# gongweibao/FleetX

Hardware: AMD Instinct MI355X
Metric: tokens/sec (whole node) GPT-3 6.7B hybrid-parallel at 1/2/4/8 MI355X (higher is better)
Workload: dtype bf16; 1 GPU; model=gpt3-6.7B, global_batch=8, seq_len=1024, parallelism=dp1, micro_batch=8, hip_graph=True, grad_reduce_dtype=float32, recompute=False

## Files before the change

csrc/kernels/norm_eltwise.hip:

```cpp
#include "fx_common.h"

namespace {

struct DropCfg {
  uint32_t klo, khi, thr;
  float scale;
  int enabled;
  const uint64_t* salt;
};

__device__ __forceinline__ DropCfg resolve_drop(DropCfg d) {
  if (d.enabled && d.salt != nullptr) {
    const uint64_t k = salt_key(((uint64_t)d.khi << 32) | d.klo, *d.salt);
    d.klo = (uint32_t)k;
    d.khi = (uint32_t)(k >> 32);
  }
  return d;
}

__device__ __forceinline__ float drop_apply(float v, uint64_t idx, const DropCfg& d) {
  if (!d.enabled) return v;
  uint32_t h = elem_rand_pair(idx, d.klo, d.khi);
  uint32_t r = (idx & 1) ? (h >> 16) : (h & 0xffffu);
  return r >= d.thr ? v * d.scale : 0.f;
// ... 129 lines not shown
      drop_apply8(v, base + c, drop);
    if (residual) {
      float r[8];
      load8<T>(residual + base + c, r);
      for (int j = 0; j < 8; ++j) v[j] += r[j];
    }
  };
  float sum = 0.f;
  for (int vi = lane; vi < nv; vi += 64) {
    float v[8];
    value(vi * 8, v);
    if (s_out) {
      store8<T>(s_out + base + vi * 8, v);
      for (int j = 0; j < 8; ++j) v[j] = round_to<T>(v[j]);
    }
    for (int j = 0; j < 8; ++j) sum += v[j];
  }
  const float mean = wave_sum(sum) / h;
  float var = 0.f;
  for (int vi = lane; vi < nv; vi += 64) {
    float v[8];
    if (s_out) load8<T>(s_out + base + vi * 8, v); else value(vi * 8, v);
    for (int j = 0; j < 8; ++j) { float d = v[j] - mean; var += d * d; }
  }
  const float rstd = rsqrtf(wave_sum(var) / h + eps);
  for (int vi = lane; vi < nv; vi += 64) {
    float v[8], g[8], b[8], o[8];
    if (s_out) load8<T>(s_out + base + vi * 8, v); else value(vi * 8, v);
    load8<T>(gamma + vi * 8, g);
    load8<T>(beta + vi * 8, b);
    for (int j = 0; j < 8; ++j) o[j] = (v[j] - mean) * rstd * g[j] + b[j];
    store8<T>(y + base + vi * 8, o);
  }
  if (lane == 0) { mean_out[row] = mean; rstd_out[row] = rstd; }
}

template <typename T, int VPT, bool MASK = false>
__global__ __launch_bounds__(256) void ln_bwd_row_kernel(
    const uint16_t* __restrict__ dy, const uint16_t* __restrict__ s,
    const float* __restrict__ mean_in, const float* __restrict__ rstd_in,
    const uint16_t* __restrict__ gamma, const uint16_t* __restrict__ ds_in,
    uint16_t* __restrict__ ds_out, uint16_t* __restrict__ dx_out, int rows, int h,
    DropCfg drop_) {
  const DropCfg drop = resolve_drop(drop_);
  const int lane = threadIdx.x & 63;
  const int row = blockIdx.x * 4 + (threadIdx.x >> 6);
  if (row >= rows) return;
  const size_t base = (size_t)row * h;
  const float mean = mean_in[row], rstd = rstd_in[row];
  float xh[VPT][8], gdy[VPT][8];
  float s1 = 0.f, s2 = 0.f;
#pragma unroll
  for (int i = 0; i < VPT; ++i) {
    const int c = (i * 64 + lane) * 8;
    if (MASK && c >= h) {
#pragma unroll
      for (int j = 0; j < 8; ++j) xh[i][j] = gdy[i][j] = 0.f;
      continue;
    }
    float a[8], g[8], d[8];
    load8<T>(s + base + c, a);
    load8<T>(gamma + c, g);
    load8<T>(dy + base + c, d);
#pragma unroll
    for (int j = 0; j < 8; ++j) {
      xh[i][j] = (a[j] - mean) * rstd;
      gdy[i][j] = d[j] * g[j];
      s1 += gdy[i][j];
      s2 += gdy[i][j] * xh[i][j];
    }
  }
  uint4 dr[VPT];
  if (ds_in) {
#pragma unroll
    for (int i = 0; i < VPT; ++i) {
      const int c = (i * 64 + lane) * 8;
      dr[i] = make_uint4(0, 0, 0, 0);
      if (!MASK || c < h) dr[i] = *reinterpret_cast<const uint4*>(ds_in + base + c);
    }
  }
  const float m1 = wave_sum(s1) / h, m2 = wave_sum(s2) / h;
#pragma unroll
  for (int i = 0; i < VPT; ++i) {
    const int c = (i * 64 + lane) * 8;
    if (MASK && c >= h) continue;
    float o[8];
#pragma unroll
    for (int j = 0; j < 8; ++j) o[j] = rstd * (gdy[i][j] - m1 - xh[i][j] * m2);
    if (ds_in) {
      float r[8];
      unpack8<T>(dr[i], r);
#pragma unroll
      for (int j = 0; j < 8; ++j) o[j] += r[j];
    }
    store8<T>(ds_out + base + c, o);
    if (drop.enabled) {
      drop_apply8(o, base + c, drop);
      store8<T>(dx_out + base + c, o);
    } else if (dx_out != ds_out) {
      store8<T>(dx_out + base + c, o);
    }
  }
}

template <typename T>
__global__ __launch_bounds__(256) void ln_bwd_row_generic(
    const uint16_t* __restrict__ dy, const uint16_t* __restrict__ s,
    const float* __restrict__ mean_in, const float* __restrict__ rstd_in,
    const uint16_t* __restrict__ gamma, const uint16_t* __restrict__ ds_in,
    uint16_t* __restrict__ ds_out, uint16_t* __restrict__ dx_out, int rows, int h,
    DropCfg drop_) {
  const DropCfg drop = resolve_drop(drop_);
  const int lane = threadIdx.x & 63;
  const int row = blockIdx.x * 4 + (threadIdx.x >> 6);
  if (row >= rows) return;
  const size_t base = (size_t)row * h;
  const float mean = mean_in[row], rstd = rstd_in[row];
  const int nv = h / 8;
  float s1 = 0.f, s2 = 0.f;
  for (int vi = lane; vi < nv; vi += 64) {
    float a[8], g[8], d[8];
    load8<T>(s + base + vi * 8, a);
    load8<T>(gamma + vi * 8, g);
    load8<T>(dy + base + vi * 8, d);
    for (int j = 0; j < 8; ++j) {
      float xh = (a[j] - mean) * rstd, gd = d[j] * g[j];
      s1 += gd;
      s2 += gd * xh;
    }
  }
  const float m1 = wave_sum(s1) / h, m2 = wave_sum(s2) / h;
  for (int vi = lane; vi < nv; vi += 64) {
    const int c = vi * 8;
    float a[8], g[8], d[8], o[8];
    load8<T>(s + base + c, a);
    load8<T>(gamma + c, g);
    load8<T>(dy + base + c, d);
    for (int j = 0; j < 8; ++j) o[j] = rstd * (d[j] * g[j] - m1 - (a[j] - mean) * rstd * m2);
    if (ds_in) {
      float r[8];
      load8<T>(ds_in + base + c, r);
      for (int j = 0; j < 8; ++j) o[j] += r[j];
    }
    store8<T>(ds_out + base + c, o);
    if (drop.enabled) {
      drop_apply8(o, base + c, drop);
      store8<T>(dx_out + base + c, o);
    } else if (dx_out != ds_out) {
      store8<T>(dx_out + base + c, o);
    }
  }
}

template <typename T, int VPT, int WPR, bool MASK, bool DB>
__global__ __launch_bounds__(256, 2) void ln_bwd_cols_kernel(
    const uint16_t* __restrict__ dy, const uint16_t* __restrict__ s,
    const float* __restrict__ mean_in, const float* __restrict__ rstd_in,
    const uint16_t* __restrict__ gamma, const uint16_t* __restrict__ ds_in,
    uint16_t* __restrict__ ds_out, uint16_t* __restrict__ dx_out, int rows, int h,
    int rows_per_group, float* __restrict__ part, DropCfg drop_) {
  constexpr int NG = 4 / WPR;
  __shared__ float red[4 * 512 * VPT];
  __shared__ float xs[2][4][2];
  const DropCfg drop = resolve_drop(drop_);
  const int lane = threadIdx.x & 63, w = threadIdx.x >> 6;
  const int grp = w / WPR, half = w % WPR;
  const int hw = h / WPR, cbase = half * hw;
  const int r0 = min(rows, (blockIdx.x * NG + grp) * rows_per_group);
  const int r1 = min(rows, r0 + rows_per_group);
  uint4 gp[VPT];
  float ag[VPT][8], ab[VPT][8], ax[DB ? VPT : 1][8];
#pragma unroll
  for (int i = 0; i < VPT; ++i) {
    const int c = (i * 64 + lane) * 8;
    gp[i] = (!MASK || c < hw) ? *reinterpret_cast<const uint4*>(gamma + cbase + c)
                              : make_uint4(0, 0, 0, 0);
#pragma unroll
    for (int j = 0; j < 8; ++j) {
      ag[i][j] = ab[i][j] = 0.f;
      if (DB) ax[i][j] = 0.f;
    }
  }
  for (int k = 0; k < rows_per_group; ++k) {
    const int r = r0 + k;
    const bool live = r < r1;
    if (WPR == 1 && !live) break;
    const size_t base = (size_t)(live ? r : 0) * h + cbase;
    uint4 ca[VPT], cd[VPT], cr[VPT];
    float mean = 0.f, rstd = 0.f, s1 = 0.f, s2 = 0.f;
    if (live) {
#pragma unroll
      for (int i = 0; i < VPT; ++i) {
        const int c = (i * 64 + lane) * 8;
        if (MASK && c >= hw) continue;
        ca[i] = *reinterpret_cast<const uint4*>(s + base + c);
        cd[i] = *reinterpret_cast<const uint4*>(dy + base + c);
      }
      if (ds_in) {
#pragma unroll
        for (int i = 0; i < VPT; ++i) {
          const int c = (i * 64 + lane) * 8;
          if (MASK && c >= hw) continue;
          cr[i] = *reinterpret_cast<const uint4*>(ds_in + base + c);
        }
      }
      mean = mean_in[r];
      rstd = rstd_in[r];
#pragma unroll
      for (int i = 0; i < VPT; ++i) {
        const int c = (i * 64 + lane) * 8;
        if (MASK && c >= hw) continue;
        float a[8], d[8], g[8];
        unpack8<T>(ca[i], a);
        unpack8<T>(cd[i], d);
        unpack8<T>(gp[i], g);
#pragma unroll
        for (int j = 0; j < 8; ++j) {
          const float xh = (a[j] - mean) * rstd, gd = d[j] * g[j];
          s1 += gd;
          s2 += gd * xh;
          ag[i][j] += d[j] * xh;
          ab[i][j] += d[j];
        }
      }
    }
    s1 = wave_sum(s1);
    s2 = wave_sum(s2);
    if constexpr (WPR > 1) {
      if (lane == 0) {
        xs[k & 1][w][0] = s1;
        xs[k & 1][w][1] = s2;
      }
      __syncthreads();
      s1 = xs[k & 1][WPR * grp][0];
      s2 = xs[k & 1][WPR * grp][1];
#pragma unroll
      for (int q = 1; q < WPR; ++q) {
        s1 += xs[k & 1][WPR * grp + q][0];
        s2 += xs[k & 1][WPR * grp + q][1];
      }
    }
    if (!live) continue;
    const float m1 = s1 / h, m2 = s2 / h;
#pragma unroll
    for (int i = 0; i < VPT; ++i) {
      const int c = (i * 64 + lane) * 8;
      if (MASK && c >= hw) continue;
      float a[8], d[8], g[8], o[8];
      unpack8<T>(ca[i], a);
      unpack8<T>(cd[i], d);
      unpack8<T>(gp[i], g);
#pragma unroll
      for (int j = 0; j < 8; ++j) o[j] = rstd * (d[j] * g[j] - m1 - (a[j] - mean) * rstd * m2);
      if (ds_in) {
        float rr[8];
        unpack8<T>(cr[i], rr);
#pragma unroll
        for (int j = 0; j < 8; ++j) o[j] += rr[j];
      }
      store8<T>(ds_out + base + c, o);
      if (drop.enabled) {
        drop_apply8(o, base + c, drop);
        store8<T>(dx_out + base + c, o);
      } else if (dx_out != ds_out) {
        store8<T>(dx_out + base + c, o);
      }
      if (DB) {
#pragma unroll
        for (int j = 0; j < 8; ++j) ax[i][j] += round_to<T>(o[j]);
      }
    }
  }
#pragma unroll
  for (int arr = 0; arr < (DB ? 3 : 2); ++arr) {
    __syncthreads();
#pragma unroll
    for (int i = 0; i < VPT; ++i) {
      const int c = (i * 64 + lane) * 8;
      if (MASK && c >= hw) continue;
#pragma unroll
      for (int j = 0; j < 8; ++j)
        red[grp * h + cbase + c + j] = arr == 0 ? ag[i][j] : arr == 1 ? ab[i][j] : ax[DB ? i : 0][j];
    }
    __syncthreads();
    float* out = part + ((size_t)arr * gridDim.x + blockIdx.x) * h;
    for (int c = threadIdx.x; c < h; c += 256) {
      float v = red[c];
#pragma unroll
      for (int q = 1; q < NG; ++q) v += red[q * h + c];
      out[c] = v;
    }
  }
}

struct LnColsOut {
  float* f32[3];
  uint16_t* t16[3];
  int acc[3];
};
template <typename T>
__global__ __launch_bounds__(256) void ln_cols_finalize_kernel(const float* __restrict__ part,
                                                               int G, int h, LnColsOut f) {
  __shared__ float tr[8][132];
  const int arr = blockIdx.y;
  const float* p = part + (size_t)arr * G * h;
  const int q = threadIdx.x & 31, sr = threadIdx.x >> 5;
  const int c0 = blockIdx.x * 128 + q * 4;
  floatx4 acc = {0.f, 0.f, 0.f, 0.f};
  if (c0 < h) {
    for (int k0 = sr; k0 < G; k0 += 128) {
      floatx4 v[16];
#pragma unroll
      for (int u = 0; u < 16; ++u) {
        const int k = k0 + 8 * u;
        v[u] = k < G ? *reinterpret_cast<const floatx4*>(p + (size_t)k * h + c0)
                     : floatx4{0.f, 0.f, 0.f, 0.f};
      }
#pragma unroll
      for (int u = 0; u < 16; ++u) acc += v[u];
    }
  }
#pragma unroll
  for (int j = 0; j < 4; ++j) tr[sr][q * 4 + j] = acc[j];
  __syncthreads();
  const int c = threadIdx.x, gc = blockIdx.x * 128 + c;
  if (c >= 128 || gc >= h) return;
  float sum = 0.f;
#pragma unroll
  for (int t = 0; t < 8; ++t) sum += tr[t][c];
  if (f.f32[arr]) f.f32[arr][gc] = f.acc[arr] ? f.f32[arr][gc] + sum : sum;
  if (f.t16[arr]) f.t16[arr][gc] = Elt<T>::from_f(sum);
}

typedef __attribute__((address_space(1))) float gf32;
typedef __attribute__((address_space(1))) int gi32;

__device__ __forceinline__ void st_part(float* p, float v) {
  __hip_atomic_store((gf32*)p, v, __ATOMIC_RELAXED, __HIP_MEMORY_SCOPE_AGENT);
}

struct ColFin {
  int* cnt;
  float* f32[2];
  uint16_t* t16[2];
  int acc[2];
};

template <typename T>
__device__ __forceinline__ void colsum_tail(const float* __restrict__ p0,
                                            const float* __restrict__ p1, int cols, int np,
                                            const ColFin& f) {
  __shared__ int last;
  asm volatile("s_waitcnt vmcnt(0)" ::: "memory");
  __syncthreads();
  if (threadIdx.x == 0) {
    const int t = __hip_atomic_fetch_add((gi32*)(f.cnt + 32 * blockIdx.x), 1, __ATOMIC_RELAXED,
                                         __HIP_MEMORY_SCOPE_AGENT);
    last = t == (int)gridDim.y - 1;
    if (last)
      __hip_atomic_store((gi32*)(f.cnt + 32 * blockIdx.x), 0, __ATOMIC_RELAXED,
                         __HIP_MEMORY_SCOPE_AGENT);
  }
  __syncthreads();
  if (!last) return;
  __builtin_amdgcn_fence(__ATOMIC_ACQUIRE, "wavefront");
  __shared__ float tr[8][132];
  const int q = threadIdx.x & 31, sr = threadIdx.x >> 5;
  const int c0 = blockIdx.x * 128 + q * 4;
  const int splits = gridDim.y;
  for (int which = 0; which < np; ++which) {
    const float* p = which ? p1 : p0;
    floatx4 s = {0.f, 0.f, 0.f, 0.f};
    if (c0 < cols) {
      const auto rs = __builtin_amdgcn_make_buffer_rsrc(const_cast<float*>(p), 0,
                                                        splits * cols * 4, 0x00020000);
      for (int k0 = sr; k0 < splits; k0 += 128) {
        floatx4 v[16];
#pragma unroll
        for (int u = 0; u < 16; ++u) {
          const int k = k0 + 8 * u;
          const uint32_t off = k < splits ? (uint32_t)(k * cols + c0) * 4u : 0x80000000u;
          v[u] = __builtin_bit_cast(floatx4, __builtin_amdgcn_raw_buffer_load_b128(rs, off, 0, 16));
        }
#pragma unroll
        for (int u = 0; u < 16; ++u) s += v[u];
      }
    }
#pragma unroll
    for (int j = 0; j < 4; ++j) tr[sr][q * 4 + j] = s[j];
    __syncthreads();
    const int c = threadIdx.x, gc = blockIdx.x * 128 + c;
    if (c < 128 && gc < cols) {
      float sum = 0.f;
#pragma unroll
      for (int t = 0; t < 8; ++t) sum += tr[t][c];
      if (f.f32[which]) f.f32[which][gc] = f.acc[which] ? f.f32[which][gc] + sum : sum;
      if (f.t16[which]) f.t16[which][gc] = Elt<T>::from_f(sum);
    }
    __syncthreads();
  }
}

template <typename T, int MODE>
__global__ __launch_bounds__(256) void coltile_partial_kernel(
    const uint16_t* __restrict__ a, const uint16_t* __restrict__ b,
    const float* __restrict__ mean, const float* __restrict__ rstd,
    float* __restrict__ p0, float* __restrict__ p1, int rows, int cols, int rows_per_split,
    ColFin fin) {
  __shared__ float red[2][16][129];
  const int tx = threadIdx.x & 15, ty = threadIdx.x >> 4;
  const int col = blockIdx.x * 128 + tx * 8;
  const int r0 = blockIdx.y * rows_per_split;
  const int r1 = min(rows, r0 + rows_per_split);
  float acc0[8], acc1[8];
#pragma unroll
  for (int j = 0; j < 8; ++j) acc0[j] = acc1[j] = 0.f;
  if (col < cols) {
    int r = r0 + ty;
    for (; r + 48 < r1; r += 64) {
      float va[4][8], vb[MODE == 0 ? 4 : 1][8], m[4], rs[4];
#pragma unroll
      for (int q = 0; q < 4; ++q) {
        const size_t off = (size_t)(r + 16 * q) * cols + col;
        load8<T>(a + off, va[q]);
        if (MODE == 0) {
          load8<T>(b + off, vb[q]);
          m[q] = mean[r + 16 * q];
          rs[q] = rstd[r + 16 * q];
        }
      }
#pragma unroll
      for (int q = 0; q < 4; ++q) {
#pragma unroll
        for (int j = 0; j < 8; ++j) {
          if (MODE == 0) {
            acc0[j] += va[q][j] * (vb[MODE == 0 ? q : 0][j] - m[q]) * rs[q];
            acc1[j] += va[q][j];
          } else {
            acc0[j] += va[q][j];
          }
        }
      }
    }
    for (; r < r1; r += 16) {
      const size_t off = (size_t)r * cols + col;
// ... 217 lines not shown
    drop_apply8(a, (uint64_t)off, drop);
    store8<T>(y + off, a);
  }
}

DropCfg make_drop(float p, uint64_t key) {
  DropCfg d;
  d.enabled = p > 0.f ? 1 : 0;
  d.klo = (uint32_t)(key & 0xffffffffu);
  d.khi = (uint32_t)(key >> 32);
  d.thr = (uint32_t)(p * 65536.0f + 0.5f);
  d.scale = p < 1.f ? 1.f / (1.f - p) : 0.f;
  d.salt = g_fx_dropout_salt;
  return d;
}

inline int grid_for(long n8) {
  long g = (n8 + 255) / 256;
  if (g > 8192) g = 8192;
  if (g < 1) g = 1;
  return (int)g;
}

inline int splits_for(int rows, int cols) {
  static const int blocks = [] {
    const char* e = getenv("FLEETX_COLSUM_BLOCKS");
    const int v = e ? atoi(e) : 0;
    return v > 0 ? v : 1024;
  }();
  int tiles = (cols + 127) / 128;
  int s = blocks / (tiles > 0 ? tiles : 1);
  if (s < 1) s = 1;
  int max_s = (rows + 15) / 16;
  if (s > max_s) s = max_s;
  if (s > 512) s = 512;
  return s;
}

}

#define FX_DISPATCH_T(dtype, ...)        \
  if (dtype == 0) {                      \
    using T = bf16;                      \
    __VA_ARGS__;                         \
  } else {                               \
    using T = f16;                       \
    __VA_ARGS__;                         \
  }

static ColFin make_fin(int* cnt, float* f0, void* t0, int acc0, float* f1, void* t1, int acc1) {
  ColFin f;
  f.cnt = cnt;
  f.f32[0] = f0; f.f32[1] = f1;
  f.t16[0] = (uint16_t*)t0; f.t16[1] = (uint16_t*)t1;
  f.acc[0] = acc0; f.acc[1] = acc1;
  return f;
}

extern "C" int fx_coltile_splits(int rows, int cols) { return splits_for(rows, cols); }

extern "C" void fx_add_ln_fwd(int dtype, const void* x, const void* bias, const void* residual,
                              const void* gamma, const void* beta, void* s_out, void* y,
                              float* mean, float* rstd, int rows, int h, float eps, float p,
                              uint64_t key, hipStream_t st) {
  DropCfg d = make_drop(p, key);
  dim3 grid((rows + 3) / 4), block(256);
  auto X = (const uint16_t*)x;
  auto B = (const uint16_t*)bias;
  auto R = (const uint16_t*)residual;
  auto G = (const uint16_t*)gamma;
  auto Be = (const uint16_t*)beta;
  auto S = (uint16_t*)s_out;
  auto Y = (uint16_t*)y;
#define LN_CASE(V)                                                                          \
  case V:                                                                                   \
    FX_DISPATCH_T(dtype, add_ln_fwd_kernel<T, V><<<grid, block, 0, st>>>(                   \
                             X, B, R, G, Be, S, Y, mean, rstd, rows, h, eps, d));           \
    break;
  if (h % 512 == 0 && h / 512 <= 16) {
    switch (h / 512) {
      LN_CASE(1) LN_CASE(2) LN_CASE(3) LN_CASE(4) LN_CASE(5) LN_CASE(6) LN_CASE(7) LN_CASE(8)
      LN_CASE(10) LN_CASE(12) LN_CASE(16)
      default:
        FX_DISPATCH_T(dtype, add_ln_fwd_generic<T><<<grid, block, 0, st>>>(
                                 X, B, R, G, Be, S, Y, mean, rstd, rows, h, eps, d));
    }
  } else if (h % 8 == 0 && h < 8 * 512) {
#define LNM_CASE(V)                                                                          \
  case V:                                                                                    \
    FX_DISPATCH_T(dtype, add_ln_fwd_kernel<T, V, true><<<grid, block, 0, st>>>(              \
                             X, B, R, G, Be, S, Y, mean, rstd, rows, h, eps, d));            \
    break;
    switch ((h + 511) / 512) {
      LNM_CASE(1) LNM_CASE(2) LNM_CASE(3) LNM_CASE(4) LNM_CASE(5) LNM_CASE(6) LNM_CASE(7)
      LNM_CASE(8)
    }
#undef LNM_CASE
  } else {
    FX_DISPATCH_T(dtype, add_ln_fwd_generic<T><<<grid, block, 0, st>>>(
                             X, B, R, G, Be, S, Y, mean, rstd, rows, h, eps, d));
  }
#undef LN_CASE
}

extern "C" void fx_ln_bwd_row(int dtype, const void* dy, const void* s, const float* mean,
                              const float* rstd, const void* gamma, const void* ds_in,
                              void* ds_out, void* dx_out, int rows, int h, float p, uint64_t key,
                              hipStream_t st) {
  DropCfg d = make_drop(p, key);
  dim3 grid((rows + 3) / 4), block(256);
  auto DY = (const uint16_t*)dy;
  auto S = (const uint16_t*)s;
  auto G = (const uint16_t*)gamma;
  auto DI = (const uint16_t*)ds_in;
  auto DS = (uint16_t*)ds_out;
  auto DX = (uint16_t*)dx_out;
#define LNB_CASE(V)                                                                       \
  case V:                                                                                 \
    FX_DISPATCH_T(dtype, ln_bwd_row_kernel<T, V><<<grid, block, 0, st>>>(                 \
                             DY, S, mean, rstd, G, DI, DS, DX, rows, h, d));              \
    break;
  if (h % 512 == 0 && h / 512 <= 8) {
    switch (h / 512) {
      LNB_CASE(1) LNB_CASE(2) LNB_CASE(3) LNB_CASE(4) LNB_CASE(5) LNB_CASE(6) LNB_CASE(7)
      LNB_CASE(8)
      default:
        FX_DISPATCH_T(dtype, ln_bwd_row_generic<T><<<grid, block, 0, st>>>(
                                 DY, S, mean, rstd, G, DI, DS, DX, rows, h, d));
    }
  } else if (h % 8 == 0 && h < 8 * 512) {
#define LNBM_CASE(V)                                                                      \
  case V:                                                                                 \
    FX_DISPATCH_T(dtype, ln_bwd_row_kernel<T, V, true><<<grid, block, 0, st>>>(           \
                             DY, S, mean, rstd, G, DI, DS, DX, rows, h, d));              \
    break;
    switch ((h + 511) / 512) {
      LNBM_CASE(1) LNBM_CASE(2) LNBM_CASE(3) LNBM_CASE(4) LNBM_CASE(5) LNBM_CASE(6)
      LNBM_CASE(7) LNBM_CASE(8)
    }
#undef LNBM_CASE
  } else {
    FX_DISPATCH_T(dtype, ln_bwd_row_generic<T><<<grid, block, 0, st>>>(
                             DY, S, mean, rstd, G, DI, DS, DX, rows, h, d));
  }
#undef LNB_CASE
}

static int ln_cols_wpr(int h) { return h <= 1536 ? 1 : h <= 3072 ? 2 : 4; }
static int ln_cols_rows_per_group(int rows, int h) {
  const int ng = 4 / ln_cols_wpr(h);
  int rpg = (rows + 512 * ng - 1) / (512 * ng);
  return rpg < 2 ? 2 : rpg;
}
extern "C" int fx_ln_bwd_cols_blocks(int rows, int h, int max_h) {
  if (rows <= 0 || h > (max_h < 4096 ? max_h : 4096) || h % (8 * ln_cols_wpr(h))) return 0;
  const int ng = 4 / ln_cols_wpr(h), rpg = ln_cols_rows_per_group(rows, h);
  return (rows + ng * rpg - 1) / (ng * rpg);
}

extern "C" int fx_ln_bwd_cols(int dtype, const void* dy, const void* s, const float* mean,
                              const float* rstd, const void* gamma, const void* ds_in,
                              void* ds_out, void* dx_out, int rows, int h, float p, uint64_t key,
                              float* part, int with_dbias, float* fg, void* tg, int accg,
                              float* fb, void* tb, int accb, float* fx, void* tx, int accx,
                              hipStream_t st) {
  const int G = fx_ln_bwd_cols_blocks(rows, h, 4096);
  if (G == 0) return -1;
  const int wpr = ln_cols_wpr(h), hw = h / wpr;
  const int rpg = ln_cols_rows_per_group(rows, h);
  DropCfg d = make_drop(p, key);
  auto DY = (const uint16_t*)dy;
  auto S = (const uint16_t*)s;
  auto GM = (const uint16_t*)gamma;
  auto DI = (const uint16_t*)ds_in;
  auto DS = (uint16_t*)ds_out;
  auto DX = (uint16_t*)dx_out;
  const int vpt = (hw + 511) / 512;
  const bool mask = hw % 512 != 0;
#define LNC_GO(V, W, M, DB)                                                                   \
  FX_DISPATCH_T(dtype, ln_bwd_cols_kernel<T, V, W, M, DB><<<G, 256, 0, st>>>(                 \
                           DY, S, mean, rstd, GM, DI, DS, DX, rows, h, rpg, part, d))
#define LNC_M(V, W)                                                                           \
  if (mask) {                                                                                 \
    if (with_dbias) { LNC_GO(V, W, true, true); } else { LNC_GO(V, W, true, false); }         \
  } else {                                                                                    \
    if (with_dbias) { LNC_GO(V, W, false, true); } else { LNC_GO(V, W, false, false); }       \
  }
#define LNC_V(V)                                                                              \
  case V:                                                                                     \
    if (wpr == 1) { LNC_M(V, 1) } else if (wpr == 2) { LNC_M(V, 2) } else { LNC_M(V, 4) }     \
    break;
  switch (vpt) {
    LNC_V(1) LNC_V(2) LNC_V(3)
    default: return -1;
  }
#undef LNC_V
#undef LNC_M
#undef LNC_GO
  LnColsOut f;
  f.f32[0] = fg; f.f32[1] = fb; f.f32[2] = fx;
  f.t16[0] = (uint16_t*)tg; f.t16[1] = (uint16_t*)tb; f.t16[2] = (uint16_t*)tx;
  f.acc[0] = accg; f.acc[1] = accb; f.acc[2] = accx;
  dim3 grid((h + 127) / 128, with_dbias ? 3 : 2);
  FX_DISPATCH_T(dtype, ln_cols_finalize_kernel<T><<<grid, 256, 0, st>>>(part, G, h, f));
  return 0;
}

extern "C" void fx_coltile_partial(int dtype, int mode, const void* a, const void* b,
                                   const float* mean, const float* rstd, float* p0, float* p1,
                                   int rows, int cols, int splits, hipStream_t st, int* cnt,
                                   float* f0, void* t0, int acc0, float* f1, void* t1, int acc1) {
  const ColFin fin = make_fin(cnt, f0, t0, acc0, f1, t1, acc1);
  int rps = (rows + splits - 1) / splits;
  dim3 grid((cols + 127) / 128, splits), block(256);
  auto A = (const uint16_t*)a;
  auto B = (const uint16_t*)b;
  if (mode == 0) {
    FX_DISPATCH_T(dtype, coltile_partial_kernel<T, 0><<<grid, block, 0, st>>>(
                             A, B, mean, rstd, p0, p1, rows, cols, rps, fin));
  } else {
    FX_DISPATCH_T(dtype, coltile_partial_kernel<T, 1><<<grid, block, 0, st>>>(
                             A, B, mean, rstd, p0, p1, rows, cols, rps, fin));
  }
}

extern "C" void fx_coltile_finalize(int dtype, const float* part, int splits, int cols,
                                    float* out_f32, void* out_t, int accumulate, hipStream_t st) {
  dim3 grid((cols + 255) / 256), block(256);
  FX_DISPATCH_T(dtype, coltile_finalize_kernel<T><<<grid, block, 0, st>>>(
                           part, splits, cols, out_f32, (uint16_t*)out_t, accumulate));
}

extern "C" void fx_bias_gelu_fwd(int dtype, int erf, const void* x, const void* bias, void* y,
                                 long n, int cols, hipStream_t st) {
  long n8 = n / 8;
  if (erf) {
    FX_DISPATCH_T(dtype, bias_gelu_fwd_kernel<T, true><<<grid_for(n8), 256, 0, st>>>(
                             (const uint16_t*)x, (const uint16_t*)bias, (uint16_t*)y, n8, cols));
  } else {
    FX_DISPATCH_T(dtype, bias_gelu_fwd_kernel<T, false><<<grid_for(n8), 256, 0, st>>>(
                             (const uint16_t*)x, (const uint16_t*)bias, (uint16_t*)y, n8, cols));
  }
}

extern "C" void fx_bias_gelu_bwd(int dtype, int erf, const void* dy, const void* x,
                                 const void* bias, void* dx, float* part, int rows, int cols,
                                 int splits, hipStream_t st, int* cnt, float* out_f32,
                                 void* out_t, int acc) {
  const ColFin fin = make_fin(cnt, out_f32, out_t, acc, nullptr, nullptr, 0);
  int rps = (rows + splits - 1) / splits;
  dim3 grid((cols + 127) / 128, splits), block(256);
  if (erf) {
    FX_DISPATCH_T(dtype, bias_gelu_bwd_kernel<T, true><<<grid, block, 0, st>>>(
                             (const uint16_t*)dy, (const uint16_t*)x, (const uint16_t*)bias,
                             (uint16_t*)dx, part, rows, cols, rps, fin));
  } else {
    FX_DISPATCH_T(dtype, bias_gelu_bwd_kernel<T, false><<<grid, block, 0, st>>>(
                             (const uint16_t*)dy, (const uint16_t*)x, (const uint16_t*)bias,
                             (uint16_t*)dx, part, rows, cols, rps, fin));
  }
}

extern "C" void fx_bias_dropout_add_fwd(int dtype, const void* x, const void* bias,
                                        const void* residual, void* out, long n, int cols, float p,
                                        uint64_t key, hipStream_t st) {
  DropCfg d = make_drop(p, key);
  long n8 = n / 8;
  FX_DISPATCH_T(dtype, bias_dropout_add_fwd_kernel<T><<<grid_for(n8), 256, 0, st>>>(
                           (const uint16_t*)x, (const uint16_t*)bias, (const uint16_t*)residual,
                           (uint16_t*)out, n8, cols, d));
}

extern "C" void fx_dropout_bwd_colsum(int dtype, const void* dout, void* dx, float* part,
                                      int rows, int cols, int splits, float p, uint64_t key,
                                      hipStream_t st, int* cnt, float* out_f32, void* out_t,
                                      int acc) {
  const ColFin fin = make_fin(cnt, out_f32, out_t, acc, nullptr, nullptr, 0);
  DropCfg d = make_drop(p, key);
  int rps = (rows + splits - 1) / splits;
  dim3 grid((cols + 127) / 128, splits), block(256);
  FX_DISPATCH_T(dtype, dropout_bwd_colsum_kernel<T><<<grid, block, 0, st>>>(
                           (const uint16_t*)dout, (uint16_t*)dx, part, rows, cols, rps, d, fin));
}

extern "C" void fx_dropout_fwd(int dtype, const void* x, void* y, long n, float p, uint64_t key,
                               hipStream_t st) {
  DropCfg d = make_drop(p, key);
  long n8 = n / 8;
  FX_DISPATCH_T(dtype, dropout_fwd_kernel<T><<<grid_for(n8), 256, 0, st>>>(
                           (const uint16_t*)x, (uint16_t*)y, n8, d));
}

const uint64_t* g_fx_dropout_salt = nullptr;
extern "C" void fx_set_dropout_salt(const void* p) {
  g_fx_dropout_salt = reinterpret_cast<const uint64_t*>(p);
}
```

fleetx_amd/ops/norm.py:

```python
import os

import torch

from . import _lib
from ..parallel import rng as _rng


_TICKETS = {}


def colsum_tickets(device, cols):
    st = torch.cuda.current_stream(device).cuda_stream
    need = 32 * ((cols + 127) // 128)
    t = _TICKETS.get(st)
    if t is None or t.numel() < need:
        t = torch.zeros(max(4096, need), dtype=torch.int32, device=device)
        _TICKETS[st] = t
    return t.data_ptr()


def _col_reduce_ln(dy, s, mean, rstd, cols, dtype):
    k = _lib.kernels()
    rows = dy.numel() // cols
    splits = k.coltile_splits(rows, cols)
    p0 = torch.empty(splits, cols, device=dy.device, dtype=torch.float32)
    p1 = torch.empty_like(p0)
    st = _lib.stream()
    dc = _lib.dt_code(dtype)
    dg = torch.empty(cols, device=dy.device, dtype=dtype)
    db = torch.empty(cols, device=dy.device, dtype=dtype)
    k.coltile_partial(dc, 0, dy.data_ptr(), s.data_ptr(), mean.data_ptr(), rstd.data_ptr(),
                      p0.data_ptr(), p1.data_ptr(), rows, cols, splits, st,
                      cnt=colsum_tickets(dy.device, cols), t0=dg.data_ptr(), t1=db.data_ptr())
    return dg, db


def _fused_param(p):
    return p is not None and getattr(p, "_fx_fused_wgrad", False) and hasattr(p, "main_grad")


def _into_main_grad(p, fill):
    from ..parallel.linear import grad_part_done
    fill(p.main_grad, not getattr(p, "_fx_fresh", False))
    p._fx_fresh = False
    grad_part_done(p)


def _col_reduce_ln_main_grad(dy, s, mean, rstd, cols, dtype, weight, lnbias):
    k = _lib.kernels()
    rows = dy.numel() // cols
    splits = k.coltile_splits(rows, cols)
    p0 = torch.empty(splits, cols, device=dy.device, dtype=torch.float32)
    p1 = torch.empty_like(p0)
    st = _lib.stream()
    dc = _lib.dt_code(dtype)
    acc = [int(not getattr(prm, "_fx_fresh", False)) for prm in (weight, lnbias)]
    k.coltile_partial(dc, 0, dy.data_ptr(), s.data_ptr(), mean.data_ptr(), rstd.data_ptr(),
                      p0.data_ptr(), p1.data_ptr(), rows, cols, splits, st,
                      cnt=colsum_tickets(dy.device, cols), f0=weight.main_grad.data_ptr(),
                      acc0=acc[0], f1=lnbias.main_grad.data_ptr(), acc1=acc[1])
    from ..parallel.linear import grad_part_done
    for prm in (weight, lnbias):
        prm._fx_fresh = False
        grad_part_done(prm)


def col_sum(x, cols):
    if not x.is_cuda:
        return x.reshape(-1, cols).float().sum(0).to(x.dtype)
    k = _lib.kernels()
    rows = x.numel() // cols
    splits = k.coltile_splits(rows, cols)
    p0 = torch.empty(splits, cols, device=x.device, dtype=torch.float32)
    st = _lib.stream()
    dc = _lib.dt_code(x.dtype)
    out = torch.empty(cols, device=x.device, dtype=x.dtype)
    k.coltile_partial(dc, 1, x.data_ptr(), 0, 0, 0, p0.data_ptr(), 0, rows, cols, splits, st,
                      cnt=colsum_tickets(x.device, cols), t0=out.data_ptr())
    return out


def col_sum_f32(x, dst, accumulate=False):
    cols = dst.numel()
    if not x.is_cuda:
        s = x.reshape(-1, cols).float().sum(0).view_as(dst)
        if accumulate:
            dst.add_(s)
        else:
            dst.copy_(s)
        return dst
    if dst.dtype != torch.float32 or not dst.is_contiguous():
        raise ValueError("col_sum_f32: dst must be contiguous fp32")
    x = x.contiguous()
    k = _lib.kernels()
    rows = x.numel() // cols
    splits = k.coltile_splits(rows, cols)
    p0 = torch.empty(splits, cols, device=x.device, dtype=torch.float32)
    st = _lib.stream()
    dc = _lib.dt_code(x.dtype)
    k.coltile_partial(dc, 1, x.data_ptr(), 0, 0, 0, p0.data_ptr(), 0, rows, cols, splits, st,
                      cnt=colsum_tickets(x.device, cols), f0=dst.data_ptr(),
                      acc0=int(accumulate))
    return dst


def _dropout_ref(x, p, key):
    if p <= 0.0:
        return x
    m = _rng.keep_mask(x.shape, p, key, x.device)
    return torch.where(m, x * (1.0 / (1.0 - p)), torch.zeros_like(x))


def _ln_bwd_cols_max_h():
    mode = os.environ.get("FLEETX_LN_BWD_FUSED", "1")
    return {"0": 0, "2": 4096}.get(mode, 1536)


def _main_grad_target(p):
    return _fused_param(p) and p.main_grad.dtype == torch.float32 and p.main_grad.is_contiguous()


def _ln_bwd_cols(k, dc, dy, s, mean, rstd, weight, ctx, ds_in, ds, dx, rows, h):
    G = k.ln_bwd_cols_blocks(rows, h, 4096)
    with_db = bool(ctx.has_bias)
    part = torch.empty(3 if with_db else 2, G, h, device=dy.device, dtype=torch.float32)
    outs, grads, done = [], [], []
    for prm, want in ((weight, True), (ctx.lnbias, True), (ctx.bias, with_db)):
        if not want:
            outs.append((0, 0, 0))
            grads.append(None)
        elif _main_grad_target(prm):
            outs.append((prm.main_grad.data_ptr(), 0, int(not getattr(prm, "_fx_fresh", False))))
            grads.append(None)
            done.append(prm)
        else:
            g = torch.empty(h, device=dy.device, dtype=dy.dtype)
            outs.append((0, g.data_ptr(), 0))
            grads.append(g)
    (fg, tg, ag), (fb, tb, ab), (fx, tx, ax) = outs
    rc = k.ln_bwd_cols(dc, dy.data_ptr(), s.data_ptr(), mean.data_ptr(), rstd.data_ptr(),
                       weight.data_ptr(), _lib.ptr(ds_in), ds.data_ptr(), dx.data_ptr(), rows, h,
                       float(ctx.p), ctx.key, part.data_ptr(), int(with_db), fg, tg, ag, fb, tb,
                       ab, fx, tx, ax, _lib.stream())
    if rc != 0:
        raise RuntimeError("ln_bwd_cols: shape rows=%d h=%d not covered" % (rows, h))
    if done:
        from ..parallel.linear import grad_part_done
        for prm in done:
            prm._fx_fresh = False
            grad_part_done(prm)
    return grads[0], grads[1], grads[2]


class _AddLayerNorm(torch.autograd.Function):
    @staticmethod
    def forward(ctx, x, bias, residual, weight, lnbias, eps, p, key, store_sum):
        h = x.shape[-1]
        rows = x.numel() // h
        ctx.p, ctx.key, ctx.has_bias, ctx.has_res = p, key, bias is not None, residual is not None
        ctx.h = h
        if x.is_cuda:
            k = _lib.kernels()
            x = x.contiguous()
            fused = bias is not None or residual is not None or p > 0
            s = torch.empty_like(x) if fused else None
            y = torch.empty_like(x)
            mean = torch.empty(rows, device=x.device, dtype=torch.float32)
            rstd = torch.empty_like(mean)
            k.add_ln_fwd(_lib.dt_code(x.dtype), x.data_ptr(), _lib.ptr(bias), _lib.ptr(residual),
                         weight.data_ptr(), lnbias.data_ptr(), _lib.ptr(s), y.data_ptr(),
                         mean.data_ptr(), rstd.data_ptr(), rows, h, float(eps), float(p), key,
                         _lib.stream())
            s_saved = s if s is not None else x
            if s is None and store_sum:
                s = x
        else:
            v = x if bias is None else x + bias
            v = _dropout_ref(v, p, key)
            if residual is not None:
                v = v + residual
            s_saved = v
            s = v if (store_sum or bias is not None or residual is not None or p > 0) else None
            vf = v.float()
            mean = vf.mean(-1).reshape(-1)
            var = ((vf - mean.view(*vf.shape[:-1], 1)) ** 2).mean(-1).reshape(-1)
            rstd = torch.rsqrt(var + eps)
            y = ((vf - mean.view(*vf.shape[:-1], 1)) * rstd.view(*vf.shape[:-1], 1) * weight.float()
                 + lnbias.float()).to(x.dtype)
        ctx.save_for_backward(s_saved, mean, rstd, weight)
        ctx.lnbias, ctx.bias = lnbias, bias
        ctx.return_sum = s is not None
        if s is None:
            return y
        return s, y

    @staticmethod
    def backward(ctx, *grads):
        if ctx.return_sum:
            ds_in, dy = grads
        else:
            ds_in, dy = None, grads[0]
        s, mean, rstd, weight = ctx.saved_tensors
        h = ctx.h
        rows = s.numel() // h
        dy = dy.contiguous()
        if ds_in is not None:
            ds_in = ds_in.contiguous()
        if dy.is_cuda:
            k = _lib.kernels()
            dc = _lib.dt_code(dy.dtype)
            ds = torch.empty_like(dy)
            dx = torch.empty_like(dy) if ctx.p > 0 else ds
            if k.ln_bwd_cols_blocks(rows, h, _ln_bwd_cols_max_h()) > 0:
                dw, db, dbias = _ln_bwd_cols(k, dc, dy, s, mean, rstd, weight, ctx, ds_in, ds, dx,
                                             rows, h)
                dres = ds if ctx.has_res else None
                return dx, dbias, dres, dw, db, None, None, None, None
            k.ln_bwd_row(dc, dy.data_ptr(), s.data_ptr(), mean.data_ptr(), rstd.data_ptr(),
                         weight.data_ptr(), _lib.ptr(ds_in), ds.data_ptr(), dx.data_ptr(), rows, h,
                         float(ctx.p), ctx.key, _lib.stream())
            if _fused_param(weight) and _fused_param(ctx.lnbias):
                _col_reduce_ln_main_grad(dy, s, mean, rstd, h, dy.dtype, weight, ctx.lnbias)
                dw = db = None
            else:
                dw, db = _col_reduce_ln(dy, s, mean, rstd, h, dy.dtype)
            dbias = None
            if ctx.has_bias:
                if _fused_param(ctx.bias):
                    _into_main_grad(ctx.bias, lambda mg, acc: col_sum_f32(dx, mg, acc))
                else:
                    dbias = col_sum(dx, h)
        else:
            sf = s.float().reshape(rows, h)
            xh = (sf - mean.view(rows, 1)) * rstd.view(rows, 1)
            g = dy.float().reshape(rows, h) * weight.float()
            m1 = g.mean(-1, keepdim=True)
            m2 = (g * xh).mean(-1, keepdim=True)
            dsf = rstd.view(rows, 1) * (g - m1 - xh * m2)
            if ds_in is not None:
                dsf = dsf + ds_in.float().reshape(rows, h)
            ds = dsf.to(dy.dtype).reshape(dy.shape)
            dx = _dropout_ref(ds, ctx.p, ctx.key)
            dw = (dy.float().reshape(rows, h) * xh).sum(0).to(weight.dtype)
            db = dy.float().reshape(rows, h).sum(0).to(weight.dtype)
            dbias = dx.float().reshape(rows, h).sum(0).to(dy.dtype) if ctx.has_bias else None
        dres = ds if ctx.has_res else None
        return dx, dbias, dres, dw, db, None, None, None, None


def add_layer_norm(x, bias, residual, weight, lnbias, eps=1e-5, p=0.0, key=0):
    return _AddLayerNorm.apply(x, bias, residual, weight, lnbias, eps, p, key, True)


def layer_norm(x, weight, bias, eps=1e-5):
    return _AddLayerNorm.apply(x, None, None, weight, bias, eps, 0.0, 0, False)


def layer_norm_keep_input(x, weight, bias, eps=1e-5):
    return _AddLayerNorm.apply(x, None, None, weight, bias, eps, 0.0, 0, True)


class FusedLayerNorm(torch.nn.Module):

    def __init__(self, hidden, eps=1e-5, dtype=None, device=None):
        super().__init__()
        self.weight = torch.nn.Parameter(torch.ones(hidden, dtype=dtype, device=device))
        self.bias = torch.nn.Parameter(torch.zeros(hidden, dtype=dtype, device=device))
        self.weight._fx_fused_wgrad_ok = True
# ... 7 lines not shown
```

Before: 28460 tokens/s.

## Add batched, prefetching multi-wave LayerNorm backward column kernel and enable it by default

Adds a separate LayerNorm backward kernel for hidden sizes that need two or four waves per row. It processes several rows per batch, so one barrier covers the cross-wave reduction for the whole batch, and it double-buffers the row loads. The fused column-reduction path now defaults to allowing hidden sizes up to 4096. For GPT-3 6.7B (h=4096) this means the fused kernel replaces the previous separate col-reduce path. In exchange it raises register pressure, which may lower occupancy, and it makes the new path the default.

```diff
diff --git a/csrc/kernels/norm_eltwise.hip b/csrc/kernels/norm_eltwise.hip
--- a/csrc/kernels/norm_eltwise.hip
+++ b/csrc/kernels/norm_eltwise.hip
@@ -305,16 +305,39 @@
   }
 }
 
-template <typename T, int VPT, int WPR, bool MASK, bool DB>
+
+template <int VPT, int NG, bool MASK>
+__device__ __forceinline__ void ln_cols_block_partial(float* __restrict__ red,
+                                                      const float (*acc)[8], int grp, int lane,
+                                                      int h, int hw, int cbase,
+                                                      float* __restrict__ part, int arr) {
+  __syncthreads();
+#pragma unroll
+  for (int i = 0; i < VPT; ++i) {
+    const int c = (i * 64 + lane) * 8;
+    if (MASK && c >= hw) continue;
+#pragma unroll
+    for (int j = 0; j < 8; ++j) red[grp * h + cbase + c + j] = acc[i][j];
+  }
+  __syncthreads();
+  float* out = part + ((size_t)arr * gridDim.x + blockIdx.x) * h;
+  for (int c = threadIdx.x; c < h; c += 256) {
+    float v = red[c];
+#pragma unroll
+    for (int q = 1; q < NG; ++q) v += red[q * h + c];
+    out[c] = v;
+  }
+}
+
+template <typename T, int VPT, bool MASK, bool DB>
 __global__ __launch_bounds__(256, 2) void ln_bwd_cols_kernel(
     const uint16_t* __restrict__ dy, const uint16_t* __restrict__ s,
     const float* __restrict__ mean_in, const float* __restrict__ rstd_in,
     const uint16_t* __restrict__ gamma, const uint16_t* __restrict__ ds_in,
     uint16_t* __restrict__ ds_out, uint16_t* __restrict__ dx_out, int rows, int h,
     int rows_per_group, float* __restrict__ part, DropCfg drop_) {
-  constexpr int NG = 4 / WPR;
+  constexpr int WPR = 1, NG = 4 / WPR;
   __shared__ float red[4 * 512 * VPT];
-  __shared__ float xs[2][4][2];
   const DropCfg drop = resolve_drop(drop_);
   const int lane = threadIdx.x & 63, w = threadIdx.x >> 6;
   const int grp = w / WPR, half = w % WPR;
@@ -379,20 +402,6 @@
     }
     s1 = wave_sum(s1);
     s2 = wave_sum(s2);
-    if constexpr (WPR > 1) {
-      if (lane == 0) {
-        xs[k & 1][w][0] = s1;
-        xs[k & 1][w][1] = s2;
-      }
-      __syncthreads();
-      s1 = xs[k & 1][WPR * grp][0];
-      s2 = xs[k & 1][WPR * grp][1];
-#pragma unroll
-      for (int q = 1; q < WPR; ++q) {
-        s1 += xs[k & 1][WPR * grp + q][0];
-        s2 += xs[k & 1][WPR * grp + q][1];
-      }
-    }
     if (!live) continue;
     const float m1 = s1 / h, m2 = s2 / h;
 #pragma unroll
@@ -444,6 +453,193 @@
       out[c] = v;
     }
   }
+}
+
+__device__ __forceinline__ void keep_packed(uint4& v) {
+  asm volatile("" : "+v"(v.x), "+v"(v.y), "+v"(v.z), "+v"(v.w));
+}
+
+template <typename T, int VPT, int WPR, bool MASK, bool DB, int RB, bool PF>
+__global__ __launch_bounds__(256, 2) void ln_bwd_cols_wide_kernel(
+    const uint16_t* __restrict__ dy, const uint16_t* __restrict__ s,
+    const float* __restrict__ mean_in, const float* __restrict__ rstd_in,
+    const uint16_t* __restrict__ gamma, const uint16_t* __restrict__ ds_in,
+    uint16_t* __restrict__ ds_out, uint16_t* __restrict__ dx_out, int rows, int h,
+    int rows_per_group, float* __restrict__ part, DropCfg drop_) {
+  static_assert(WPR == 2 || WPR == 4, "one wave per row: ln_bwd_cols_kernel");
+  constexpr int NG = 4 / WPR;
+  __shared__ float red[4 * 512 * VPT];
+  __shared__ __attribute__((aligned(16))) float xs[2][RB][4][2];
+  const DropCfg drop = resolve_drop(drop_);
+  const int lane = threadIdx.x & 63, w = __builtin_amdgcn_readfirstlane(threadIdx.x >> 6);
+  const int grp = w / WPR, half = w % WPR;
+  const int hw = h / WPR, cbase = half * hw;
+  const int r0 = min(rows, (blockIdx.x * NG + grp) * rows_per_group);
+  const int r1 = min(rows, r0 + rows_per_group);
+  uint4 gp[VPT];
+  float ag[VPT][8], ab[VPT][8], ax[DB ? VPT : 1][8];
+#pragma unroll
+  for (int i = 0; i < VPT; ++i) {
+    const int c = (i * 64 + lane) * 8;
+    gp[i] = (!MASK || c < hw) ? *reinterpret_cast<const uint4*>(gamma + cbase + c)
+                              : make_uint4(0, 0, 0, 0);
+#pragma unroll
+    for (int j = 0; j < 8; ++j) {
+      ag[i][j] = ab[i][j] = 0.f;
+      if (DB) ax[i][j] = 0.f;
+    }
+  }
+  struct Batch {
+    uint4 ca[RB][VPT], cd[RB][VPT], cr[RB][VPT];
+    float mean[RB], rstd[RB];
+    bool live[RB];
+    size_t base[RB];
+  };
+  auto load = [&](Batch& t, int b) {
+#pragma unroll
+    for (int q = 0; q < RB; ++q) {
+      const int r = r0 + b * RB + q;
+      t.live[q] = r < r1;
+      const int rr = t.live[q] ? r : 0;
+      t.base[q] = (size_t)rr * h + cbase;
+#pragma unroll
+      for (int i = 0; i < VPT; ++i) {
+        const int c = (i * 64 + lane) * 8;
+        if (MASK && c >= hw) continue;
+        t.ca[q][i] = *reinterpret_cast<const uint4*>(s + t.base[q] + c);
+        t.cd[q][i] = *reinterpret_cast<const uint4*>(dy + t.base[q] + c);
+      }
+      t.mean[q] = mean_in[rr];
+      t.rstd[q] = rstd_in[rr];
+    }
+    if (ds_in) {
+#pragma unroll
+      for (int q = 0; q < RB; ++q) {
+#pragma unroll
+        for (int i = 0; i < VPT; ++i) {
+          const int c = (i * 64 + lane) * 8;
+          if (MASK && c >= hw) continue;
+          t.cr[q][i] = *reinterpret_cast<const uint4*>(ds_in + t.base[q] + c);
+        }
+      }
+    }
+  };
+  auto run = [&](Batch& t, int b) {
+    float s1[RB], s2[RB];
+#pragma unroll
+    for (int i = 0; i < VPT; ++i) keep_packed(gp[i]);
+#pragma unroll
+    for (int q = 0; q < RB; ++q) {
+      s1[q] = s2[q] = 0.f;
+      if (t.live[q]) {
+#pragma unroll
+        for (int i = 0; i < VPT; ++i) {
+          const int c = (i * 64 + lane) * 8;
+          if (MASK && c >= hw) continue;
+          float a[8], d[8], g[8];
+          unpack8<T>(t.ca[q][i], a);
+          unpack8<T>(t.cd[q][i], d);
+          unpack8<T>(gp[i], g);
+#pragma unroll
+          for (int j = 0; j < 8; ++j) {
+            const float xh = (a[j] - t.mean[q]) * t.rstd[q], gd = d[j] * g[j];
+            s1[q] += gd;
+            s2[q] += gd * xh;
+            ag[i][j] += d[j] * xh;
+            ab[i][j] += d[j];
+          }
+        }
+      }
+      __builtin_amdgcn_sched_barrier(0);
+    }
+#pragma unroll
+    for (int q = 0; q < RB; ++q) {
+      s1[q] = wave_sum(s1[q]);
+      s2[q] = wave_sum(s2[q]);
+    }
+    if (lane == 0) {
+#pragma unroll
+      for (int q = 0; q < RB; ++q) {
+        xs[b & 1][q][w][0] = s1[q];
+        xs[b & 1][q][w][1] = s2[q];
+      }
+    }
+    __syncthreads();
+#pragma unroll
+    for (int q = 0; q < RB; ++q) {
+      s1[q] = xs[b & 1][q][WPR * grp][0];
+      s2[q] = xs[b & 1][q][WPR * grp][1];
+#pragma unroll
+      for (int u = 1; u < WPR; ++u) {
+        s1[q] += xs[b & 1][q][WPR * grp + u][0];
+        s2[q] += xs[b & 1][q][WPR * grp + u][1];
+      }
+    }
+#pragma unroll
+    for (int q = 0; q < RB; ++q) {
+#pragma unroll
+      for (int i = 0; i < VPT; ++i) {
+        keep_packed(t.ca[q][i]);
+        keep_packed(t.cd[q][i]);
+      }
+    }
+#pragma unroll
+    for (int q = 0; q < RB; ++q) {
+      if (t.live[q]) {
+        const float mean = t.mean[q], rstd = t.rstd[q];
+        const float m1 = s1[q] / h, m2 = s2[q] / h;
+#pragma unroll
+        for (int i = 0; i < VPT; ++i) {
+          const int c = (i * 64 + lane) * 8;
+          if (MASK && c >= hw) continue;
+          float a[8], d[8], g[8], o[8];
+          unpack8<T>(t.ca[q][i], a);
+          unpack8<T>(t.cd[q][i], d);
+          unpack8<T>(gp[i], g);
+#pragma unroll
+          for (int j = 0; j < 8; ++j) o[j] = rstd * (d[j] * g[j] - m1 - (a[j] - mean) * rstd * m2);
+          if (ds_in) {
+            float rr[8];
+            unpack8<T>(t.cr[q][i], rr);
+#pragma unroll
+            for (int j = 0; j < 8; ++j) o[j] += rr[j];
+          }
+          store8<T>(ds_out + t.base[q] + c, o);
+          if (drop.enabled) {
+            drop_apply8(o, t.base[q] + c, drop);
+            store8<T>(dx_out + t.base[q] + c, o);
+          } else if (dx_out != ds_out) {
+            store8<T>(dx_out + t.base[q] + c, o);
+          }
+          if (DB) {
+#pragma unroll
+            for (int j = 0; j < 8; ++j) ax[i][j] += round_to<T>(o[j]);
+          }
+        }
+      }
+      __builtin_amdgcn_sched_barrier(0);
+    }
+  };
+  const int nb = (rows_per_group + RB - 1) / RB;
+  if constexpr (PF) {
+    Batch t0, t1;
+    load(t0, 0);
+    for (int b = 0; b < nb; b += 2) {
+      load(t1, b + 1);
+      run(t0, b);
+      load(t0, b + 2);
+      run(t1, b + 1);
+    }
+  } else {
+    for (int b = 0; b < nb; ++b) {
+      Batch t;
+      load(t, b);
+      run(t, b);
+    }
+  }
+  ln_cols_block_partial<VPT, NG, MASK>(red, ag, grp, lane, h, hw, cbase, part, 0);
+  ln_cols_block_partial<VPT, NG, MASK>(red, ab, grp, lane, h, hw, cbase, part, 1);
+  if constexpr (DB) ln_cols_block_partial<VPT, NG, MASK>(red, ax, grp, lane, h, hw, cbase, part, 2);
 }
 
 struct LnColsOut {
@@ -967,6 +1163,9 @@
   int rpg = (rows + 512 * ng - 1) / (512 * ng);
   return rpg < 2 ? 2 : rpg;
 }
+#ifndef FX_LN_COLS_RB
+#define FX_LN_COLS_RB 2
+#endif
 extern "C" int fx_ln_bwd_cols_blocks(int rows, int h, int max_h) {
   if (rows <= 0 || h > (max_h < 4096 ? max_h : 4096) || h % (8 * ln_cols_wpr(h))) return 0;
   const int ng = 4 / ln_cols_wpr(h), rpg = ln_cols_rows_per_group(rows, h);
@@ -992,26 +1191,32 @@
   auto DX = (uint16_t*)dx_out;
   const int vpt = (hw + 511) / 512;
   const bool mask = hw % 512 != 0;
-#define LNC_GO(V, W, M, DB)                                                                   \
-  FX_DISPATCH_T(dtype, ln_bwd_cols_kernel<T, V, W, M, DB><<<G, 256, 0, st>>>(                 \
-                           DY, S, mean, rstd, GM, DI, DS, DX, rows, h, rpg, part, d))
-#define LNC_M(V, W)                                                                           \
+#define LNC_ARGS DY, S, mean, rstd, GM, DI, DS, DX, rows, h, rpg, part, d
+#define LNC_ONE(V, W, M, DB)                                                                  \
+  FX_DISPATCH_T(dtype, ln_bwd_cols_kernel<T, V, M, DB><<<G, 256, 0, st>>>(LNC_ARGS))
+#define LNC_WIDE(V, W, M, DB)                                                                 \
+  FX_DISPATCH_T(dtype, ln_bwd_cols_wide_kernel<T, V, W, M, DB, FX_LN_COLS_RB, (V < 3)>     \
+                           <<<G, 256, 0, st>>>(LNC_ARGS))
+#define LNC_M(GO, V, W)                                                                       \
   if (mask) {                                                                                 \
-    if (with_dbias) { LNC_GO(V, W, true, true); } else { LNC_GO(V, W, true, false); }         \
+    if (with_dbias) { GO(V, W, true, true); } else { GO(V, W, true, false); }                 \
   } else {                                                                                    \
-    if (with_dbias) { LNC_GO(V, W, false, true); } else { LNC_GO(V, W, false, false); }       \
-  }
-#define LNC_V(V)                                                                              \
-  case V:                                                                                     \
-    if (wpr == 1) { LNC_M(V, 1) } else if (wpr == 2) { LNC_M(V, 2) } else { LNC_M(V, 4) }     \
-    break;
-  switch (vpt) {
-    LNC_V(1) LNC_V(2) LNC_V(3)
+    if (with_dbias) { GO(V, W, false, true); } else { GO(V, W, false, false); }               \
+  }
+  const int inst = wpr * 10 + vpt;
+  switch (inst) {
+    case 11: LNC_M(LNC_ONE, 1, 1) break;
+    case 12: LNC_M(LNC_ONE, 2, 1) break;
+    case 13: LNC_M(LNC_ONE, 3, 1) break;
+    case 22: LNC_M(LNC_WIDE, 2, 2) break;
+    case 23: LNC_M(LNC_WIDE, 3, 2) break;
+    case 42: LNC_M(LNC_WIDE, 2, 4) break;
     default: return -1;
   }
-#undef LNC_V
 #undef LNC_M
-#undef LNC_GO
+#undef LNC_WIDE
+#undef LNC_ONE
+#undef LNC_ARGS
   LnColsOut f;
   f.f32[0] = fg; f.f32[1] = fb; f.f32[2] = fx;
   f.t16[0] = (uint16_t*)tg; f.t16[1] = (uint16_t*)tb; f.t16[2] = (uint16_t*)tx;
diff --git a/fleetx_amd/ops/norm.py b/fleetx_amd/ops/norm.py
--- a/fleetx_amd/ops/norm.py
+++ b/fleetx_amd/ops/norm.py
@@ -112,8 +112,8 @@
 
 
 def _ln_bwd_cols_max_h():
-    mode = os.environ.get("FLEETX_LN_BWD_FUSED", "1")
-    return {"0": 0, "2": 4096}.get(mode, 1536)
+    mode = os.environ.get("FLEETX_LN_BWD_FUSED", "2")
+    return {"0": 0, "1": 1536}.get(mode, 4096)
 
 
 def _main_grad_target(p):
```

Measured after the change: 28540 tokens/s (median of 6 runs). About the same (+0.3%).
